# Melthizar/RRTE

Measured on AMD Instinct MI355X. Metric: Mray/s (primary+shadow) at 1920x1080, sdf-showcase scene; 1/2/4/8 GPU, higher is better.
Workload: dtype f32; 1 GPU; sdf-showcase 1920x1080, lambert_shadow, spp=1, max_depth=1, pixel-centre jitter; scene=sdf-showcase, width=1920, height=1080, mode=lambert_shadow, primary_rays_per_frame=2073600, frames_in_flight=4, hw_queues=32, parallelism=single

## Files before the change

rrte_amd/csrc/jit.hip:

```cpp
#include <hip/hip_runtime.h>
#include <hip/hiprtc.h>

#include <chrono>
#include <cinttypes>
#include <cstdio>
#include <cstdlib>
#include <cstring>
#include <mutex>
#include <sys/stat.h>
#include <unistd.h>
#include <string>
#include <vector>

#include "jit.hpp"

namespace rrte {
namespace {

#include "jit_headers.inc"

void emit_f(std::string& s, float v) {
    char buf[48];
    if (v != v) {
        snprintf(buf, sizeof buf, "__builtin_nanf(\"\")");
    } else if (v == __builtin_huge_valf()) {
        snprintf(buf, sizeof buf, "__builtin_huge_valf()");
    } else if (v == -__builtin_huge_valf()) {
        snprintf(buf, sizeof buf, "(-__builtin_huge_valf())");
    } else {
        snprintf(buf, sizeof buf, "%af", (double)v);
    }
    s += buf;
}

void emit_fa(std::string& s, const float* v, int n) {
    s += "{";
    for (int i = 0; i < n; ++i) {
        if (i) s += ",";
        emit_f(s, v[i]);
    }
    s += "}";
}

void emit_u(std::string& s, uint32_t v) { s += std::to_string(v) + "u"; }

}

static std::string full_scene_arrays(const DPrim* prims, uint32_t np, const DMaterial* mats, uint32_t nm,
                                     const DLight* lights, uint32_t nl, const rrte_sdf_node* nodes, uint32_t nn);
static void append_kernel(std::string& s, const rrte_sdf_node* nodes, uint32_t nn, int mode, bool cull, bool single,
                          bool topo);

std::string jit_source(const DPrim* prims, uint32_t np, const DMaterial* mats, uint32_t nm, const DLight* lights,
                       uint32_t nl, const rrte_sdf_node* nodes, uint32_t nn, int mode, bool cull, bool single,
                       const JitTopo* topo) {
    std::string s;
    s.reserve(8192 + np * 600 + nn * 200);
    s += "typedef __hip_internal::uint8_t uint8_t;\ntypedef __hip_internal::uint32_t uint32_t;\n"
         "typedef __hip_internal::int32_t int32_t;\ntypedef __hip_internal::uint64_t uint64_t;\n"
         "#include \"ray_kernels.hpp\"\n#define RRTE_JIT_BLOCK 64\n"
         "namespace rrte_jit {\nstruct Scene {\n  static constexpr bool kStatic = true, kTopo = ";
    s += topo ? "true;\n" : "false;\n";
    s += "  static constexpr uint32_t num_prims = " + std::to_string(np) + "u, num_lights = " + std::to_string(nl) +
         "u, num_materials = " + std::to_string(nm) + "u;\n";
    if (topo) {
        s += "  static constexpr rrte::TopoPrim topo_prims[" + std::to_string(np ? np : 1) + "] = {";
        for (uint32_t i = 0; i < np; ++i) {
            s += i ? ",{" : "{";
            emit_u(s, prims[i].kind); s += ",";
            emit_u(s, prims[i].sdf_first); s += ",";
            emit_u(s, prims[i].sdf_count); s += ",";
            s += topo->convex[i] ? "true}" : "false}";
        }
        if (!np) s += "{}";
        s += "};\n  static constexpr rrte::TopoNode topo_nodes[" + std::to_string(nn ? nn : 1) + "] = {";
        for (uint32_t i = 0; i < nn; ++i) {
            s += i ? ",{" : "{";
            emit_u(s, nodes[i].op); s += ",{";
            emit_u(s, nodes[i].i[0]); s += ",";
            emit_u(s, nodes[i].i[1]); s += ",";
            emit_u(s, nodes[i].i[2]); s += "}}";
        }
        if (!nn) s += "{}";
        s += "};\n  static constexpr rrte::TopoLight topo_lights[" + std::to_string(nl ? nl : 1) + "] = {";
        for (uint32_t i = 0; i < nl; ++i) {
            s += i ? ",{" : "{";
            emit_u(s, lights[i].kind); s += ",";
            s += topo->cullable[i] ? "true}" : "false}";
        }
        if (!nl) s += "{}";
        s += "};\n  const rrte::DPrim* prims;\n  const rrte::DMaterial* mats;\n  const rrte::DLight* lights;\n"
             "  const rrte_sdf_node* nodes;\n";
    } else {
        s += full_scene_arrays(prims, np, mats, nm, lights, nl, nodes, nn);
    }
    s += "  rrte::MeshView mesh;  // runtime mesh buffers (kernel argument)\n};\n}  // namespace rrte_jit\n";
    append_kernel(s, nodes, nn, mode, cull, single, topo != nullptr);
    return s;
}

static std::string full_scene_arrays(const DPrim* prims, uint32_t np, const DMaterial* mats, uint32_t nm,
                              const DLight* lights, uint32_t nl, const rrte_sdf_node* nodes, uint32_t nn) {
    std::string s;
    s += "  static constexpr rrte::DPrim prims[" + std::to_string(np ? np : 1) + "] = {";
    for (uint32_t i = 0; i < np; ++i) {
        const DPrim& p = prims[i];
        s += i ? ",\n    {" : "\n    {";
        emit_u(s, p.kind); s += ",";
        s += std::to_string(p.material) + ",";
        emit_u(s, p.sdf_first); s += ",";
        emit_u(s, p.sdf_count); s += ",";
        emit_u(s, p.sdf_max_steps); s += ",";
        emit_f(s, p.sdf_step_scale); s += ",";
        emit_f(s, p.sdf_hit_eps); s += ",";
        emit_u(s, p.flags); s += ",";
        emit_fa(s, p.p, 20); s += ",";
        emit_fa(s, p.xf, 12); s += ",";
        emit_fa(s, p.inv, 12); s += ",{}}";
    }
    if (!np) s += "{}";
    s += "};\n  static constexpr rrte::DMaterial mats[" + std::to_string(nm ? nm : 1) + "] = {";
    for (uint32_t i = 0; i < nm; ++i) {
        const DMaterial& m = mats[i];
        s += i ? ",{" : "{";
        emit_u(s, m.kind); s += ",";
        emit_f(s, m.fuzz); s += ",";
        emit_f(s, m.ior); s += ",0.0f,";
        emit_fa(s, m.albedo, 4); s += "}";
    }
    if (!nm) s += "{}";
    s += "};\n  static constexpr rrte::DLight lights[" + std::to_string(nl ? nl : 1) + "] = {";
    for (uint32_t i = 0; i < nl; ++i) {
        const DLight& l = lights[i];
        s += i ? ",{" : "{";
        emit_u(s, l.kind); s += ",";
        const float sc[7] = {l.intensity, l.range, l.linear, l.quadratic, l.inner_angle, l.outer_angle, 0.0f};
        for (int k = 0; k < 7; ++k) { emit_f(s, sc[k]); s += ","; }
        emit_fa(s, l.position, 4); s += ",";
        emit_fa(s, l.direction, 4); s += ",";
        emit_fa(s, l.color, 4); s += ",";
        emit_fa(s, l.cI, 4); s += "}";
    }
    if (!nl) s += "{}";
    s += "};\n  static constexpr rrte_sdf_node nodes[" + std::to_string(nn ? nn : 1) + "] = {";
    for (uint32_t i = 0; i < nn; ++i) {
        const rrte_sdf_node& n = nodes[i];
        s += i ? ",{" : "{";
        emit_u(s, n.op); s += ",{";
        emit_u(s, n.i[0]); s += ",";
        emit_u(s, n.i[1]); s += ",";
        emit_u(s, n.i[2]); s += "},";
        emit_fa(s, n.f, 12); s += "}";
    }
    if (!nn) s += "{}";
    s += "};\n";
    return s;
}

static void append_kernel(std::string& s, const rrte_sdf_node* nodes, uint32_t nn, int mode, bool cull, bool single,
                   bool topo) {
    int min_waves = 8;
    if (const char* w = getenv("RRTE_JIT_MIN_WAVES"); w && *w) min_waves = atoi(w);
    std::string lb = "RRTE_JIT_BLOCK";
    if (min_waves > 0) lb += ", " + std::to_string(min_waves);
    auto entry = [&](const char* name, const char* traits) {
        s += "extern \"C\" __global__ __launch_bounds__(" + lb + ") void " + name + "(rrte::KParams kp, rrte::Cull cl, "
             "rrte::MeshView mv, uint32_t* __restrict__ o8, float4* __restrict__ of, unsigned long long* __restrict__ ctr, "
             "rrte::SceneValues sv) {\n"
             "  rrte::ray_kernel_body<" + std::to_string(mode) + ", rrte_jit::Scene, " + (single ? "true" : "false") + ", " +
             (cull ? "true" : "false") + ", " + traits + ">(kp, rrte_jit::Scene{" +
             (topo ? "sv.prims, sv.mats, sv.lights, sv.nodes, mv" : "mv") + "}, cl, o8, of, ctr);\n}\n";
    };
    entry("rrte_jit_kernel", "rrte::LaunchAny");
    if (single && !topo) entry("rrte_jit_kernel_plain", "rrte::LaunchPlain");
}

static std::vector<std::string> rtc_options() {
    std::vector<std::string> opts = {"--offload-arch=gfx950", "-O1", "-ffp-contract=off", "-std=c++17", "-Wno-pass-failed",
                                     "-mllvm", "-amdgpu-sched-strategy=max-ilp"};
    if (const char* e = getenv("RRTE_JIT_EXTRA_OPTS")) {
        std::string t;
        for (const char* c = e;; ++c) {
            if (*c == ' ' || *c == 0) {
                if (!t.empty()) opts.push_back(t);
                t.clear();
                if (*c == 0) break;
            } else {
                t += *c;
            }
        }
    }
    return opts;
}

static bool rtc_compile(const std::string& src, std::vector<char>& code, std::string& log) {
    if (const char* dump = getenv("RRTE_JIT_DUMP")) {
        if (FILE* f = fopen(dump, "w")) {
            fwrite(src.data(), 1, src.size(), f);
            fclose(f);
        }
    }
    static const std::string scene_hdr = [] {
        std::string h = kHdrDeviceScene;
        const std::string from = "#include \"../../include/rrte_hip.h\"";
        const size_t at = h.find(from);
        if (at != std::string::npos) h.replace(at, from.size(), "#include \"rrte_hip.h\"");
        return h;
    }();
    const char* hdrs[] = {kHdrApi, scene_hdr.c_str(), kHdrRayKernels};
    const char* names[] = {"rrte_hip.h", "device_scene.hpp", "ray_kernels.hpp"};
    hiprtcProgram prog;
    if (hiprtcCreateProgram(&prog, src.c_str(), "rrte_scene_jit.hip", 3, hdrs, names) != HIPRTC_SUCCESS) {
        log = "hiprtcCreateProgram failed";
        return false;
    }
    const std::vector<std::string> sopts = rtc_options();
    std::vector<const char*> opts;
    for (const std::string& o : sopts) opts.push_back(o.c_str());
    hiprtcResult r = hiprtcCompileProgram(prog, (int)opts.size(), opts.data());
    size_t ls = 0;
    hiprtcGetProgramLogSize(prog, &ls);
    if (ls > 1) {
        std::vector<char> l(ls + 1, 0);
        hiprtcGetProgramLog(prog, l.data());
        log.assign(l.data());
    }
    if (r != HIPRTC_SUCCESS) {
        hiprtcDestroyProgram(&prog);
        if (log.empty()) log = hiprtcGetErrorString(r);
        return false;
    }
    size_t cs = 0;
    hiprtcGetCodeSize(prog, &cs);
    code.resize(cs);
    hiprtcGetCode(prog, code.data());
    hiprtcDestroyProgram(&prog);
    return true;
}

bool jit_compile_only(const std::string& src, std::string& log) {
    std::vector<char> code;
    return rtc_compile(src, code, log);
}

namespace {

uint64_t fnv1a(const std::string& s, uint64_t h) {
    for (unsigned char c : s) {
        h ^= c;
        h *= 0x100000001b3ull;
    }
    return h;
}

std::string cache_dir() {
    if (const char* e = getenv("RRTE_JIT_CACHE"); e && e[0] == '0') return "";
    if (const char* d = getenv("RRTE_JIT_CACHE_DIR"); d && *d) return d;
    if (const char* x = getenv("XDG_CACHE_HOME"); x && *x) return std::string(x) + "/rrte-jit";
    if (const char* h = getenv("HOME"); h && *h) return std::string(h) + "/.cache/rrte-jit";
    return "";
}

struct CacheKey {
    uint64_t a, b, len;
    std::string name;
};

const std::string& headers_digest() {
    static const std::string d = [] {
        std::string all;
        for (const char* h : {kHdrApi, kHdrDeviceScene, kHdrRayKernels}) {
            all += h;
            all += '\0';
        }
        char buf[64];
        snprintf(buf, sizeof buf, "%016" PRIx64 "%016" PRIx64 ":%zu", fnv1a(all, 0xcbf29ce484222325ull),
                 fnv1a(all, 0x84222325cbf29ce4ull), all.size());
        return std::string(buf);
    }();
    return d;
}

}

std::string jit_cache_name(const std::string& src, const char* hdr_override);

namespace {

CacheKey cache_key(const std::string& src, const char* hdr_override = nullptr) {
    int maj = 0, min = 0;
    hiprtcVersion(&maj, &min);
    std::string all = src;
    all += "\n//headers:";
    if (hdr_override) all += std::to_string(fnv1a(hdr_override, 0xcbf29ce484222325ull));
    else all += headers_digest();
    all += "\n//opts:";
    for (const std::string& o : rtc_options()) {
        all += o;
        all += '\x1f';
    }
    all += "//hiprtc " + std::to_string(maj) + "." + std::to_string(min);
    CacheKey k{fnv1a(all, 0xcbf29ce484222325ull), fnv1a(all, 0x84222325cbf29ce4ull), (uint64_t)all.size(), ""};
    char buf[64];
    snprintf(buf, sizeof buf, "%016" PRIx64 "%016" PRIx64, k.a, k.b);
    k.name = buf;
    return k;
}

bool cache_load(const std::string& dir, const CacheKey& k, std::vector<char>& code) {
    FILE* f = fopen((dir + "/" + k.name + ".hsaco").c_str(), "rb");
    if (!f) return false;
    uint64_t hdr[4] = {};
    bool ok = fread(hdr, sizeof hdr, 1, f) == 1 && hdr[0] == k.a && hdr[1] == k.b && hdr[2] == k.len && hdr[3] > 0 &&
              hdr[3] < (256ull << 20);
    if (ok) {
        code.resize(hdr[3]);
        ok = fread(code.data(), 1, code.size(), f) == code.size();
    }
    fclose(f);
    return ok;
}

void cache_store(const std::string& dir, const CacheKey& k, const std::vector<char>& code) {
    std::string cur;
    for (size_t i = 0; i <= dir.size(); ++i) {
        if (i == dir.size() || dir[i] == '/') {
            if (!cur.empty()) (void)mkdir(cur.c_str(), 0755);
        }
        if (i < dir.size()) cur += dir[i];
    }
    const std::string tmp = dir + "/." + k.name + "." + std::to_string((long)getpid()) + ".tmp";
    FILE* f = fopen(tmp.c_str(), "wb");
    if (!f) return;
    const uint64_t hdr[4] = {k.a, k.b, k.len, (uint64_t)code.size()};
    const bool ok = fwrite(hdr, sizeof hdr, 1, f) == 1 && fwrite(code.data(), 1, code.size(), f) == code.size();
    if (fclose(f) == 0 && ok) (void)rename(tmp.c_str(), (dir + "/" + k.name + ".hsaco").c_str());
    else (void)remove(tmp.c_str());
}

}

std::string jit_cache_name(const std::string& src, const char* hdr_override) { return cache_key(src, hdr_override).name; }

JitCode jit_compile_code(const std::string& src) {
    static std::mutex mu;
    std::lock_guard<std::mutex> lock(mu);
    JitCode jc;
    const auto t0 = std::chrono::steady_clock::now();
    const std::string dir = cache_dir();
    const CacheKey key = cache_key(src);
    if (!dir.empty() && cache_load(dir, key, jc.code)) {
        jc.ok = true;
        jc.from_cache = true;
    } else {
        jc.ok = rtc_compile(src, jc.code, jc.log);
        if (jc.ok && !dir.empty()) cache_store(dir, key, jc.code);
    }
    jc.compile_ms = std::chrono::duration<double, std::milli>(std::chrono::steady_clock::now() - t0).count();
    return jc;
}

bool jit_load(const JitCode& jc, JitKernel& out, std::string& log) {
    if (!jc.ok) {
        log = jc.log;
        return false;
    }
    hipError_t e = hipModuleLoadData(&out.module, jc.code.data());
    if (e != hipSuccess) {
        log = std::string("hipModuleLoadData: ") + hipGetErrorString(e);
        return false;
    }
    e = hipModuleGetFunction(&out.fn, out.module, "rrte_jit_kernel");
    if (e != hipSuccess) {
        log = std::string("hipModuleGetFunction: ") + hipGetErrorString(e);
        (void)hipModuleUnload(out.module);
        out.module = nullptr;
        return false;
    }
    if (hipModuleGetFunction(&out.fn_plain, out.module, "rrte_jit_kernel_plain") != hipSuccess) {
        out.fn_plain = nullptr;
        (void)hipGetLastError();
    }
    out.code_bytes = jc.code.size();
    out.compile_ms = jc.compile_ms;
    out.from_cache = jc.from_cache;
    return true;
}

bool jit_compile(const std::string& src, JitKernel& out, std::string& log) {
    return jit_load(jit_compile_code(src), out, log);
}

void jit_release(JitKernel& k) {
    if (k.module) (void)hipModuleUnload(k.module);
    k.module = nullptr;
    k.fn = nullptr;
    k.fn_plain = nullptr;
}

}
```

Before: 118,000 Mray/s.

## Add grouped primitive search with mask-based group skipping to JIT kernel

Adds compile-time unrolled closest-hit and occlusion searches that walk primitives in fixed-size groups. Each group is tested against a per-ray primitive mask so that whole groups can be skipped. The occlusion path stops testing once every lane of the wavefront has found a hit. It also narrows the mask type to 32 bits for small scenes. The aim is to cut per-ray intersection work and divergence, at the cost of extra mask branches and larger unrolled code.

```diff
diff --git a/rrte_amd/csrc/jit.hip b/rrte_amd/csrc/jit.hip
--- a/rrte_amd/csrc/jit.hip
+++ b/rrte_amd/csrc/jit.hip
@@ -18,6 +18,7 @@
 namespace {
 
 #include "jit_headers.inc"
+#include "jit_search.inc"
 
 void emit_f(std::string& s, float v) {
     char buf[48];
@@ -95,6 +96,7 @@
         s += full_scene_arrays(prims, np, mats, nm, lights, nl, nodes, nn);
     }
     s += "  rrte::MeshView mesh;  // runtime mesh buffers (kernel argument)\n};\n}  // namespace rrte_jit\n";
+    s += kSrcSearchGroups;
     append_kernel(s, nodes, nn, mode, cull, single, topo != nullptr);
     return s;
 }
diff --git a/rrte_amd/csrc/search_groups.hpp b/rrte_amd/csrc/search_groups.hpp
--- /dev/null
+++ b/rrte_amd/csrc/search_groups.hpp
@@ -0,0 +1,98 @@
+#ifndef RRTE_SEARCH_GROUPS
+#define RRTE_SEARCH_GROUPS 6
+#endif
+#if RRTE_SEARCH_GROUPS > 0
+namespace rrte {
+namespace search {
+
+constexpr uint32_t kGroup = RRTE_SEARCH_GROUPS;
+
+template <bool NARROW> struct MaskOf { typedef uint64_t type; };
+template <> struct MaskOf<true> { typedef uint32_t type; };
+
+template <class M>
+constexpr M bits_of(uint32_t lo, uint32_t hi) {
+    M m = 0;
+    for (uint32_t i = lo; i < hi && i < 8u * sizeof(M); ++i) m |= (M)1 << i;
+    return m;
+}
+
+template <uint32_t I, uint32_t E, bool SOLO, class S, class M>
+__device__ __forceinline__ void occluded_objects(const S& sc, const Ray& r, float t_min, float t_max, M& mask, int self,
+                                                 bool& hit_any) {
+    if constexpr (I < E) {
+        if (SOLO ? true : I >= 8u * sizeof(M) ? mask != 0 : ((mask >> I) & (M)1) != 0) {
+            Hit h;
+            if (!hit_any && (int)I != self && any_hit_at(sc, UC<I>{}, r, t_min, t_max, h)) hit_any = true;
+            if (__all(hit_any)) mask = 0;
+        }
+        occluded_objects<I + 1u, E, SOLO>(sc, r, t_min, t_max, mask, self, hit_any);
+    }
+}
+template <uint32_t G, class S, class M>
+__device__ __forceinline__ void occluded_groups(const S& sc, const Ray& r, float t_min, float t_max, M& mask, int self,
+                                                bool& hit_any) {
+    constexpr uint32_t lo = G * kGroup, hi = lo + kGroup < S::num_prims ? lo + kGroup : S::num_prims;
+    if constexpr (lo < S::num_prims) {
+        constexpr M gbits = bits_of<M>(lo, hi);
+        if (hi > 8u * sizeof(M) ? mask != 0 : (mask & gbits) != 0)
+            occluded_objects<lo, hi, hi - lo == 1u>(sc, r, t_min, t_max, mask, self, hit_any);
+        occluded_groups<G + 1u>(sc, r, t_min, t_max, mask, self, hit_any);
+    }
+}
+
+struct Best {
+    int idx;
+    float t;
+    uint32_t sub;
+};
+template <uint32_t I, uint32_t E, bool SOLO, class S>
+__device__ __forceinline__ void closest_objects(const S& sc, const Ray& r, float t_min, uint32_t pmask, Best& b) {
+    if constexpr (I < E) {
+        if (SOLO || I >= 32u || ((pmask >> I) & 1u) != 0u) {
+            Hit h;
+            h.sub = 0u;
+            float tmax = (prim_at(sc, UC<I>{}).kind == RRTE_PRIM_SDF && b.idx >= 0) ? b.t : kInf;
+            if (intersect_at<false>(sc, UC<I>{}, r, t_min, tmax, h)) {
+                if (b.idx < 0 || h.t < b.t || (h.t == b.t && (int)I < b.idx)) {
+                    b.t = h.t;
+                    b.sub = h.sub;
+                    b.idx = (int)I;
+                }
+            }
+        }
+        closest_objects<I + 1u, E, SOLO>(sc, r, t_min, pmask, b);
+    }
+}
+template <uint32_t G, class S>
+__device__ __forceinline__ void closest_groups(const S& sc, const Ray& r, float t_min, uint32_t pmask, Best& b) {
+    constexpr uint32_t lo = G * kGroup, hi = lo + kGroup < S::num_prims ? lo + kGroup : S::num_prims;
+    if constexpr (lo < S::num_prims) {
+        constexpr uint32_t gbits = bits_of<uint32_t>(lo, hi);
+        if (hi > 32u || (pmask & gbits) != 0u) closest_objects<lo, hi, hi - lo == 1u>(sc, r, t_min, pmask, b);
+        closest_groups<G + 1u>(sc, r, t_min, pmask, b);
+    }
+}
+
+}
+
+__device__ __forceinline__ int closest_t(const rrte_jit::Scene& sc, const Ray& r, float t_min, float& best_t,
+                                         uint32_t& best_sub, uint32_t pmask = ~0u) {
+    search::Best b{-1, kInf, 0u};
+    search::closest_groups<0u>(sc, r, t_min, pmask, b);
+    best_t = b.t;
+    best_sub = b.sub;
+    return b.idx;
+}
+
+__device__ __forceinline__ bool occluded(const rrte_jit::Scene& sc, const Ray& r, float t_min, float t_max, uint64_t mask,
+                                         int self = -1) {
+    typedef search::MaskOf<(rrte_jit::Scene::num_prims <= 32u)>::type M;
+    bool hit_any = false;
+    M m = (M)mask;
+    search::occluded_groups<0u>(sc, r, t_min, t_max, m, self, hit_any);
+    return hit_any;
+}
+
+}
+#endif
```

After: 124,500 Mray/s (median of 6 runs). 1.05x the previous value.
